# peach-xiao/EMRT

Measured on AMD Instinct MI355X. Metric: training tiles/sec at 256x256, higher is better.
Workload: dtype bf16; 1 GPU; EMRT ResNet50, Potsdam 256x256, 6 classes, batch 8 per GPU, fwd+bwd+SGD step (BASELINE configs[1]), bf16; global_batch=8, parallelism=dp1, hipgraph=True

## Files before the change

emrt_amd/csrc/common.hpp:

```cpp
#pragma once
#include <hip/hip_runtime.h>
#include <stdint.h>
#include <stdio.h>
#include <string.h>

#define EMRT_F32 0
#define EMRT_BF16 1
#define EMRT_F16 2

namespace emrt {

extern thread_local char g_err[512];
inline int fail(const char* fn, const char* msg) {
  snprintf(g_err, sizeof(g_err), "%s: %s", fn, msg);
  return -1;
}
inline int check_launch(const char* fn) {
  hipError_t e = hipGetLastError();
  if (e != hipSuccess) {
    snprintf(g_err, sizeof(g_err), "%s: launch failed: %s", fn, hipGetErrorString(e));
    return -2;
  }
  return 0;
}
#define EMRT_REQUIRE(cond, msg) \
  do {                          \
    if (!(cond)) return emrt::fail(__func__, msg); \
  } while (0)

struct Tuning {
  int conv_tile;
  int wgrad_split;
  int thin_cblk;
  int thin_blocks;
  int thin_ch;
  int no_thin_bwd;
  int igemm64_nst;
  int wgrad_nst;
  int pair_max;
  int msda_fwd_global;
  int msda_bwd_global;
  int msda_lds_min_pairs;
  int msda_bwd_dref_lds;
  int msda_band_halo;
  int msda_scatter_qsplit;
  int msda_scatter_cuts;
  int msda_fwd_chunks;
  int msda_fwd_threads;
  int msda_fwd_probe;
  int bn_block_kb;
  int bn_operand_blocks;
  int ln_bwd_rows;
  int ln_bwd_max_blocks;
  int ln_bwd_threads;
  int ln_atomic;
  int gn_group_blocks;
  int gn_stat_rows;
  int gn_bwd_stat_rows;
  int gn_apply_rows;
  int igemm8p_probe;
  int igemm8p_cmajor;
  int igemm8p_min_blocks;
  int wgrad8p_min_steps;
  int wgrad8p_slab;
  int wgrad8p_xcd;
  int wgrad8p_force;
  int no_ksplit128;
  int wgrad_no_overwrite;
  int no_s2_dgrad;
  int wgroup_blocks;
  int wgroup_min_steps;
  int wgroup_max;
  int wgroup8;
  int wgroup8_blocks;
  int wgroup8_min_work;
  int msda_scatter_merge;
  int msda_scatter_mfma;
  int msda_mf_bands;
  int sgd_nt;
  int mha_bwd_split;
  int mha_valu;
  int no_bna;
  int memcpy_kernel;
  int xk;
};
extern Tuning g_tune;

struct Scratch {
  void* ptr; size_t bytes; void* stream;
  unsigned* tick;
  float* xk_part;
};
constexpr size_t SCRATCH_TICK_BYTES = 65536;
constexpr int SCRATCH_TICKS = (int)(SCRATCH_TICK_BYTES / 4);
constexpr size_t SCRATCH_XK_BYTES = 8u << 20;
extern Scratch g_scratch;

struct bf16_t {
  unsigned short v;
};
struct f16_t {
  unsigned short v;
};

__device__ __forceinline__ float to_f32(float x) { return x; }
__device__ __forceinline__ float to_f32(bf16_t x) { return __uint_as_float(((uint32_t)x.v) << 16); }
__device__ __forceinline__ float to_f32(f16_t x) { return (float)__builtin_bit_cast(_Float16, x.v); }
__device__ __forceinline__ float bf16_bits_to_f32(uint32_t lo16) { return __uint_as_float(lo16 << 16); }
__device__ __forceinline__ float f16_bits_to_f32(uint32_t lo16) { return (float)__builtin_bit_cast(_Float16, (unsigned short)lo16); }

template <class T>
__device__ __forceinline__ T from_f32(float f);
template <>
__device__ __forceinline__ float from_f32<float>(float f) {
  return f;
}
template <>
__device__ __forceinline__ bf16_t from_f32<bf16_t>(float f) {
  __bf16 b = (__bf16)f;
  bf16_t r;
  r.v = __builtin_bit_cast(unsigned short, b);
  return r;
}
template <>
__device__ __forceinline__ f16_t from_f32<f16_t>(float f) {
  f16_t r;
  r.v = __builtin_bit_cast(unsigned short, (_Float16)f);
  return r;
}
typedef __attribute__((ext_vector_type(2))) _Float16 emrt_half2_t;
typedef __attribute__((ext_vector_type(2))) float emrt_float2_t;
__device__ __forceinline__ uint32_t pack_f16x2(float lo, float hi) {
  emrt_half2_t h = __builtin_convertvector((emrt_float2_t){lo, hi}, emrt_half2_t);
  return __builtin_bit_cast(uint32_t, h);
}
__device__ __forceinline__ void unpack_f16x2(uint32_t w, float& lo, float& hi) {
  const emrt_half2_t h = __builtin_bit_cast(emrt_half2_t, w);
  lo = (float)h.x;
  hi = (float)h.y;
}
__device__ __forceinline__ uint32_t pack_bf16x2(float lo, float hi) {
  return (uint32_t)from_f32<bf16_t>(lo).v | ((uint32_t)from_f32<bf16_t>(hi).v << 16);
}

template <class T>
struct Vec4;
template <>
struct Vec4<float> {
  __device__ static __forceinline__ void load(const float* p, float (&o)[4]) {
    float4 v = *reinterpret_cast<const float4*>(p);
    o[0] = v.x; o[1] = v.y; o[2] = v.z; o[3] = v.w;
  }
  __device__ static __forceinline__ void store(float* p, const float (&o)[4]) {
    *reinterpret_cast<float4*>(p) = make_float4(o[0], o[1], o[2], o[3]);
  }
};
template <>
struct Vec4<bf16_t> {
  __device__ static __forceinline__ void load(const bf16_t* p, float (&o)[4]) {
    uint2 v = *reinterpret_cast<const uint2*>(p);
    o[0] = bf16_bits_to_f32(v.x & 0xffffu); o[1] = __uint_as_float(v.x & 0xffff0000u);
    o[2] = bf16_bits_to_f32(v.y & 0xffffu); o[3] = __uint_as_float(v.y & 0xffff0000u);
  }
  __device__ static __forceinline__ void store(bf16_t* p, const float (&o)[4]) {
    uint2 v;
    v.x = pack_bf16x2(o[0], o[1]);
    v.y = pack_bf16x2(o[2], o[3]);
    *reinterpret_cast<uint2*>(p) = v;
  }
};

template <>
struct Vec4<f16_t> {
  __device__ static __forceinline__ void load(const f16_t* p, float (&o)[4]) {
    uint2 v = *reinterpret_cast<const uint2*>(p);
    unpack_f16x2(v.x, o[0], o[1]);
    unpack_f16x2(v.y, o[2], o[3]);
  }
  __device__ static __forceinline__ void store(f16_t* p, const float (&o)[4]) {
    uint2 v;
    v.x = pack_f16x2(o[0], o[1]);
    v.y = pack_f16x2(o[2], o[3]);
    *reinterpret_cast<uint2*>(p) = v;
  }
};

template <class T>
struct Vec8;
template <>
struct Vec8<float> {
  __device__ static __forceinline__ void load(const float* p, float (&o)[8]) {
    float4 a = *reinterpret_cast<const float4*>(p), b = *reinterpret_cast<const float4*>(p + 4);
    o[0] = a.x; o[1] = a.y; o[2] = a.z; o[3] = a.w; o[4] = b.x; o[5] = b.y; o[6] = b.z; o[7] = b.w;
  }
  __device__ static __forceinline__ void store(float* p, const float (&o)[8]) {
    *reinterpret_cast<float4*>(p) = make_float4(o[0], o[1], o[2], o[3]);
    *reinterpret_cast<float4*>(p + 4) = make_float4(o[4], o[5], o[6], o[7]);
  }
};
template <>
struct Vec8<bf16_t> {
  __device__ static __forceinline__ void unpack(const uint4& v, float (&o)[8]) {
    uint32_t w[4] = {v.x, v.y, v.z, v.w};
#pragma unroll
    for (int i = 0; i < 4; ++i) {
      o[2 * i] = bf16_bits_to_f32(w[i] & 0xffffu);
      o[2 * i + 1] = __uint_as_float(w[i] & 0xffff0000u);
    }
  }
  __device__ static __forceinline__ void load(const bf16_t* p, float (&o)[8]) {
    uint4 v = *reinterpret_cast<const uint4*>(p);
    uint32_t w[4] = {v.x, v.y, v.z, v.w};
#pragma unroll
    for (int i = 0; i < 4; ++i) {
      o[2 * i] = bf16_bits_to_f32(w[i] & 0xffffu);
      o[2 * i + 1] = __uint_as_float(w[i] & 0xffff0000u);
    }
  }
  __device__ static __forceinline__ void store(bf16_t* p, const float (&o)[8]) {
    uint4 v;
    v.x = pack_bf16x2(o[0], o[1]); v.y = pack_bf16x2(o[2], o[3]);
    v.z = pack_bf16x2(o[4], o[5]); v.w = pack_bf16x2(o[6], o[7]);
    *reinterpret_cast<uint4*>(p) = v;
  }
};

template <>
struct Vec8<f16_t> {
// ... 92 lines not shown
```

emrt_amd/csrc/conv.hip:

```cpp
#include "common.hpp"
#include "bn_operand.hpp"
#include <stdlib.h>
#include <type_traits>

using namespace emrt;

typedef __attribute__((ext_vector_type(8))) __bf16 bf16x8_t;
typedef __attribute__((ext_vector_type(4))) short short4_t;
typedef __attribute__((ext_vector_type(16))) float f32x16_t;

struct ConvArgs {
  const void* in;
  const void* w;
  void* out;
  const float* bias;
  const float* scale;
  const void* res;
  int N, H, W, C, ldin;
  long long in_bs;
  int OH, OW, OC, ldout;
  long long out_bs;
  int ldres;
  long long res_bs;
  int KH, KW, stride, pad;
// ... 2024 lines not shown
  BwdGroupArgs g;
  bool groupable = true;
  long long total = 0;
  for (int i = 0; i < n; ++i) {
    const EmrtConvBwdDesc& b = descs[i];
    ConvArgs& d = g.d[i];
    d.in = b.dy; d.w = b.w_bwd_packed; d.out = b.dx; d.bias = nullptr; d.scale = nullptr; d.res = b.accumulate ? b.dx : nullptr;
    d.N = b.N; d.H = b.OH; d.W = b.OW; d.C = b.OC; d.ldin = b.lddy; d.in_bs = b.dy_bs;
    d.OH = b.H; d.OW = b.W; d.OC = b.C; d.ldout = b.lddx; d.out_bs = b.dx_bs;
    d.ldres = b.accumulate ? b.lddx : 0; d.res_bs = b.accumulate ? b.dx_bs : 0;
    d.KH = b.KH; d.KW = b.KW; d.stride = b.stride; d.pad = b.pad; d.dil = 1; d.relu = 0; d.out_f32 = 0; d.cmajor = 0; d.stats = nullptr;
    d.mask_y = nullptr; d.ldy = 0; d.y_bs = 0; d.mask_scale = 1.f; d.stat_x = nullptr; d.ldsx = 0; d.sx_bs = 0;
    d.xk_S = 0; d.xk_part = nullptr; d.xk_tick = nullptr; d.drop_seed = nullptr; d.drop_salt = 0; d.drop_p = 0.f;
    WgradArgs& w = g.w[i];
    w.x = b.x; w.dy = b.dy; w.dw = b.dw;
    w.N = b.N; w.H = b.H; w.W = b.W; w.C = b.C; w.ldx = b.ldx; w.x_bs = b.x_bs;
    w.OH = b.OH; w.OW = b.OW; w.OC = b.OC; w.lddy = b.lddy; w.dy_bs = b.dy_bs;
    w.KH = b.KH; w.KW = b.KW; w.stride = b.stride; w.pad = b.pad; w.dil = 1; w.tiles_per_split = 0; w.dbias = b.dbias; w.overwrite = 0;
    const bool vec = conv_desc_is_vec<T>(d) && wgrad_is_vec<T>(w) && d.OC > 32;
    groupable = groupable && vec;
    int tx = 1, ty = 1, S = 1;
    if (vec) wgrad_plan<T>(w, tx, ty, S);
    const long long Md = (long long)d.N * d.OH * d.OW;
    g.nd[i] = (int)(((Md + 63) / 64) * ((d.OC + 63) / 64));
    g.wtx[i] = tx; g.wty[i] = ty;
    g.first[i] = (int)total;
    total += g.nd[i] + (long long)tx * ty * S;
  }
  for (int i = n; i <= EMRT_MAX_GROUP; ++i) g.first[i] = (int)total;
  for (int i = n; i < EMRT_MAX_GROUP; ++i) { g.d[i] = g.d[0]; g.w[i] = g.w[0]; g.nd[i] = 0; g.wtx[i] = 1; g.wty[i] = 1; }
  if (!groupable || total > 4096) {
    for (int i = 0; i < n; ++i) {
      const int rc = conv_bwd_dispatch<T>(g.d[i], g.w[i], st);
      if (rc) return rc;
    }
    return 0;
  }
  auto kern = bwd_group_kernel<T>;
  const size_t lds_d = (size_t)2 * 128 * 144, lds_w = (size_t)4 * Cfg::BKM * Cfg::PITCH;
  const size_t lds = lds_d > lds_w ? lds_d : lds_w;
  static bool attr_done = false;
  if (!attr_done) {
    if (hipFuncSetAttribute(reinterpret_cast<const void*>(kern), hipFuncAttributeMaxDynamicSharedMemorySize, (int)lds) != hipSuccess)
      return fail("emrt_conv2d_bwd_group", "cannot raise the dynamic LDS limit");
    attr_done = true;
  }
  hipLaunchKernelGGL(kern, dim3((unsigned)total), dim3(256), lds, st, g);
  return check_launch("emrt_conv2d_bwd_group");
}

extern "C" int emrt_conv2d_bwd_group(const EmrtConvBwdDesc* descs, int n, int dtype, void* stream) {
  EMRT_REQUIRE(descs && n >= 1 && n <= EMRT_MAX_GROUP, "1..6 problems");
  EMRT_REQUIRE_TRAIN_DTYPE(dtype);
  for (int i = 0; i < n; ++i) {
    const EmrtConvBwdDesc& b = descs[i];
    EMRT_REQUIRE(b.x && b.dy && b.w_bwd_packed && b.dx, "null pointer");
    EMRT_REQUIRE((b.dw == nullptr) == (descs[0].dw == nullptr) && (b.dw || !b.dbias), "dw == NULL (data gradients only) must hold for every problem of the group, without dbias");
    EMRT_REQUIRE(b.N > 0 && b.H > 0 && b.W > 0 && b.C > 0 && b.OC > 0 && b.KH > 0 && b.KW > 0 && b.stride > 0 && b.pad >= 0, "bad dims");
    EMRT_REQUIRE(b.OH == (b.H + 2 * b.pad - b.KH) / b.stride + 1 && b.OW == (b.W + 2 * b.pad - b.KW) / b.stride + 1, "output size mismatch");
    EMRT_REQUIRE((long long)b.N * b.OH * b.OW + 512 < (1ll << 31) && (long long)b.N * b.H * b.W + 512 < (1ll << 31), "more than 2^31 pixels");
    EMRT_REQUIRE(b.lddx >= b.C && b.dx_bs >= 0, "bad dx strides");
    const long long esz = dtype == EMRT_F32 ? 4 : 2;
    const long long x_ext = ((long long)(b.N - 1) * b.x_bs + ((long long)b.H * b.W - 1) * b.ldx + b.C) * esz;
    const long long dy_ext = ((long long)(b.N - 1) * b.dy_bs + ((long long)b.OH * b.OW - 1) * b.lddy + b.OC) * esz;
    EMRT_REQUIRE(b.x_bs >= 0 && b.dy_bs >= 0 && x_ext < (1ll << 31) && dy_ext < (1ll << 31), "operand spans 2 GiB or more");
    EMRT_REQUIRE((long long)b.H * b.W < (1 << 24) && (long long)b.ldx * esz < (1 << 24) && b.stride < (1 << 12), "map too large for the 24-bit address arithmetic");
  }
  hipStream_t st = (hipStream_t)stream;
  return dtype == EMRT_F32 ? conv_bwd_group_dispatch<float>(descs, n, st) : conv_bwd_group_dispatch<bf16_t>(descs, n, st);
}

struct EmrtConvDgradDesc {
  const void* dy; const void* w_bwd_packed; void* dx; int lddx; long long dx_bs; int accumulate;
  int N, H, W, C, OH, OW, OC, lddy; long long dy_bs; int KH, KW, stride, pad, dilation;
  double* bn_stats; const void* mask_y; int ldy; long long y_bs; float mask_scale; const void* stat_x; int ldsx; long long sx_bs;
  const void* addend; int ldadd; long long add_bs;
};

static void dgrad_args_from_desc(ConvArgs& d, const EmrtConvDgradDesc& b) {
  d.in = b.dy; d.w = b.w_bwd_packed; d.out = b.dx; d.bias = nullptr; d.scale = nullptr; d.res = nullptr;
  d.N = b.N; d.H = b.OH; d.W = b.OW; d.C = b.OC; d.ldin = b.lddy; d.in_bs = b.dy_bs;
  d.OH = b.H; d.OW = b.W; d.OC = b.C; d.ldout = b.lddx; d.out_bs = b.dx_bs;
  d.ldres = 0; d.res_bs = 0;
  if (b.accumulate) { d.res = b.dx; d.ldres = b.lddx; d.res_bs = b.dx_bs; }
  else if (b.addend) { d.res = b.addend; d.ldres = b.ldadd; d.res_bs = b.add_bs; }
  d.KH = b.KH; d.KW = b.KW; d.stride = b.stride; d.pad = b.pad; d.dil = b.dilation; d.relu = 0; d.out_f32 = 0; d.cmajor = g_tune.igemm8p_cmajor; d.stats = b.bn_stats;
  d.mask_y = b.mask_y; d.ldy = b.ldy; d.y_bs = b.y_bs; d.mask_scale = b.mask_scale; d.stat_x = b.stat_x; d.ldsx = b.ldsx; d.sx_bs = b.sx_bs;
  d.xk_S = 0; d.xk_part = nullptr; d.xk_tick = nullptr; d.drop_seed = nullptr; d.drop_salt = 0; d.drop_p = 0.f;
}

template <class T>
static int conv_dgrad_multi_dispatch(const EmrtConvDgradDesc* descs, int n, hipStream_t st) {
  ConvGroupArgs g;
  bool groupable = n >= 2;
  long long total = 0;
  for (int i = 0; i < n; ++i) {
    ConvArgs& d = g.p[i];
    dgrad_args_from_desc(d, descs[i]);
    const long long Md = (long long)d.N * d.OH * d.OW;
    const long long nb = ((Md + 63) / 64) * ((d.OC + 63) / 64);
    g.first[i] = (int)total;
    total += nb;
    groupable = groupable && conv_desc_is_vec<T>(d) && d.OC > 32 && nb <= 2048;
  }
  for (int i = n; i <= EMRT_MAX_GROUP; ++i) g.first[i] = (int)total;
  for (int i = n; i < EMRT_MAX_GROUP; ++i) g.p[i] = g.p[0];
  if (!groupable || total > 4096) {
    for (int i = 0; i < n; ++i) {
      const int rc = conv_dispatch<T, 1>(g.p[i], st);
      if (rc) return rc;
    }
    return 0;
  }
  hipLaunchKernelGGL((igemm_group_kernel<T, 1>), dim3((unsigned)total), dim3(256), (size_t)2 * 128 * 144, st, g);
  return check_launch("emrt_conv2d_dgrad_multi");
}

extern "C" int emrt_conv2d_dgrad_multi(const EmrtConvDgradDesc* descs, int n, int dtype, void* stream) {
  EMRT_REQUIRE(descs && n >= 1 && n <= EMRT_MAX_GROUP, "1..6 problems");
  EMRT_REQUIRE_TRAIN_DTYPE(dtype);
  for (int i = 0; i < n; ++i) {
    const EmrtConvDgradDesc& b = descs[i];
    EMRT_REQUIRE(b.dy && b.w_bwd_packed && b.dx, "null pointer");
    EMRT_REQUIRE(b.N > 0 && b.H > 0 && b.W > 0 && b.C > 0 && b.OH > 0 && b.OW > 0 && b.OC > 0, "bad dims");
    EMRT_REQUIRE(b.KH > 0 && b.KW > 0 && b.stride > 0 && b.pad >= 0 && b.dilation >= 1, "bad kernel geometry");
    EMRT_REQUIRE(b.OH == (b.H + 2 * b.pad - b.dilation * (b.KH - 1) - 1) / b.stride + 1 && b.OW == (b.W + 2 * b.pad - b.dilation * (b.KW - 1) - 1) / b.stride + 1, "output size mismatch");
    EMRT_REQUIRE((long long)b.N * b.OH * b.OW + 512 < (1ll << 31) && (long long)b.N * b.H * b.W + 512 < (1ll << 31), "more than 2^31 pixels (32-bit pixel arithmetic)");
    const long long esz = dtype == EMRT_F32 ? 4 : 2;
    const long long dy_ext = ((long long)(b.N - 1) * b.dy_bs + ((long long)b.OH * b.OW - 1) * b.lddy + b.OC) * esz;
    const long long w_ext = (long long)b.OC * b.KH * b.KW * b.C * esz;
    EMRT_REQUIRE(b.dy_bs >= 0 && dy_ext < (1ll << 31) && w_ext < (1ll << 31), "operand spans 2 GiB or more (32-bit buffer offsets)");
    EMRT_REQUIRE((long long)b.OH * b.OW < (1 << 24) && (long long)b.lddy * esz < (1 << 24) && b.stride < (1 << 12), "map too large for the 24-bit address arithmetic");
    EMRT_REQUIRE(b.lddx >= b.C && b.dx_bs >= 0, "bad dx strides");
    EMRT_REQUIRE(!(b.accumulate && b.addend), "accumulate adds into dx itself; addend is a different tensor");
    EMRT_REQUIRE(!b.stat_x || b.mask_y, "stat_x replaces the mask tensor in the second statistic: it needs mask_y");
    for (int j = 0; j < i; ++j) EMRT_REQUIRE(descs[j].dx != b.dx, "two problems of one launch must not write the same dx");
  }
  hipStream_t st = (hipStream_t)stream;
  return dtype == EMRT_F32 ? conv_dgrad_multi_dispatch<float>(descs, n, st) : conv_dgrad_multi_dispatch<bf16_t>(descs, n, st);
}

#define EMRT_MAX_WGROUP 24
struct EmrtWgradDesc {
  const void* x; const void* dy; float* dw; float* dbias;
  int N, H, W, C, ldx; long long x_bs;
  int OH, OW, OC, lddy; long long dy_bs;
  int KH, KW, stride, pad, dilation;
  int dw_is_zero;
};
struct WgradGroupArgs {
  WgradArgs w[EMRT_MAX_WGROUP];
  int first[EMRT_MAX_WGROUP + 1];
  short wtx[EMRT_MAX_WGROUP], wty[EMRT_MAX_WGROUP];
  int n, xcd;
};

template <class T>
__global__ __launch_bounds__(256, 2) void wgrad_group_kernel(WgradGroupArgs g) {
  extern __shared__ __attribute__((aligned(16))) unsigned char smem_all[];
  const int nb = g.first[g.n];
  int w = (int)blockIdx.x;
  if (g.xcd) {
    const int k = w & 7, idx = w >> 3;
    const int w0 = (int)(((long long)k * nb) >> 3), w1 = (int)(((long long)(k + 1) * nb) >> 3);
    w = w0 + idx;
    if (w >= w1) return;
  } else if (w >= nb) return;
  int i = 0;
  for (int k = 1; k < g.n; ++k) i += w >= g.first[k] ? 1 : 0;
  i = __builtin_amdgcn_readfirstlane(i);
  const int local = w - g.first[i];
  const int tx = g.wtx[i], ty = g.wty[i];
  const int bz = __builtin_amdgcn_readfirstlane(local / (tx * ty)), t = __builtin_amdgcn_readfirstlane(local - bz * (tx * ty));
  const int by = __builtin_amdgcn_readfirstlane(t / tx);
  wgrad_body<T, true, 1>(g.w[i], __builtin_amdgcn_readfirstlane(t - by * tx), by, bz, smem_all);
}

static void wgrad_args_from_desc(WgradArgs& a, const EmrtWgradDesc& d) {
  a.x = d.x; a.dy = d.dy; a.dw = d.dw;
  a.N = d.N; a.H = d.H; a.W = d.W; a.C = d.C; a.ldx = d.ldx; a.x_bs = d.x_bs;
  a.OH = d.OH; a.OW = d.OW; a.OC = d.OC; a.lddy = d.lddy; a.dy_bs = d.dy_bs;
  a.KH = d.KH; a.KW = d.KW; a.stride = d.stride; a.pad = d.pad; a.dil = d.dilation; a.tiles_per_split = 0; a.dbias = d.dbias;
  a.overwrite = d.dw_is_zero ? 1 : 0;
}

template <class T>
static int wgrad_group_dispatch(const EmrtWgradDesc* descs, int n, hipStream_t st) {
  using Cfg = WgradCfg<T>;
  WgradArgs pend[EMRT_MAX_WGROUP];
  int npend = 0;
  auto flush = [&]() -> int {
    if (npend == 0) return 0;
    if (npend == 1) { const int rc = wgrad_dispatch<T>(pend[0], st); npend = 0; return rc; }
    int tx[EMRT_MAX_WGROUP], ty[EMRT_MAX_WGROUP], S1[EMRT_MAX_WGROUP];
    long long mt[EMRT_MAX_WGROUP], work = 0;
    for (int i = 0; i < npend; ++i) {
      WgradArgs tmp = pend[i];
      wgrad_plan<T>(tmp, tx[i], ty[i], S1[i]);
      mt[i] = ((long long)pend[i].N * pend[i].OH * pend[i].OW + Cfg::BKM - 1) / Cfg::BKM;
      work += (long long)tx[i] * ty[i] * mt[i];
    }
    int order[EMRT_MAX_WGROUP];
    long long tps[EMRT_MAX_WGROUP], Sl[EMRT_MAX_WGROUP];
    {
      long long Tt = (work + g_tune.wgroup_blocks - 1) / (g_tune.wgroup_blocks > 0 ? g_tune.wgroup_blocks : 1024);
      if (Tt < g_tune.wgroup_min_steps) Tt = g_tune.wgroup_min_steps;
      if (Tt < 1) Tt = 1;
      for (int i = 0; i < npend; ++i) {
        long long S = (mt[i] + Tt - 1) / Tt;
        Sl[i] = S > S1[i] ? S1[i] : (S < 1 ? 1 : S);
      }
    }
    for (int i = 0; i < npend; ++i) {
      tps[i] = (mt[i] + Sl[i] - 1) / Sl[i];
      order[i] = i;
    }
    for (int i = 1; i < npend; ++i)
      for (int j = i; j > 0 && tps[order[j]] > tps[order[j - 1]]; --j) { const int t_ = order[j]; order[j] = order[j - 1]; order[j - 1] = t_; }
    WgradGroupArgs g;
    long long total = 0;
    for (int q = 0; q < npend; ++q) {
      const int i = order[q];
      g.w[q] = pend[i];
      g.w[q].tiles_per_split = (int)tps[i];
      const long long S = (mt[i] + tps[i] - 1) / tps[i];
      if (S > 1 || g_tune.wgrad_no_overwrite) g.w[q].overwrite = 0;
      g.first[q] = (int)total;
      g.wtx[q] = (short)tx[i]; g.wty[q] = (short)ty[i];
      total += (long long)tx[i] * ty[i] * S;
    }
    for (int q = npend; q <= EMRT_MAX_WGROUP; ++q) g.first[q] = (int)total;
    for (int q = npend; q < EMRT_MAX_WGROUP; ++q) { g.w[q] = g.w[0]; g.wtx[q] = 1; g.wty[q] = 1; }
    g.n = npend; g.xcd = g_tune.wgrad8p_xcd;
    npend = 0;
    if (total >= (1ll << 30)) return fail("emrt_conv2d_wgrad_group", "too many blocks");
    auto kern = wgrad_group_kernel<T>;
    const size_t lds = (size_t)4 * Cfg::BKM * Cfg::PITCH;
    static bool attr_done = false;
    if (!attr_done) {
      if (hipFuncSetAttribute(reinterpret_cast<const void*>(kern), hipFuncAttributeMaxDynamicSharedMemorySize, (int)lds) != hipSuccess)
        return fail("emrt_conv2d_wgrad_group", "cannot raise the dynamic LDS limit");
      attr_done = true;
    }
    hipLaunchKernelGGL(kern, dim3(8u * (unsigned)((total + 7) / 8)), dim3(256), lds, st, g);
    return check_launch("emrt_conv2d_wgrad_group");
  };
  WgradArgs pend8[EMRT_MAX_WGROUP8];
  int npend8 = 0;
  auto flush8 = [&]() -> int {
    if (npend8 == 0) return 0;
    const int rc = launch_wgrad8p_group(pend8, npend8, st);
    npend8 = 0;
    return rc;
  };
  auto aliased = [&](int i) { for (int j = 0; j < n; ++j) if (j != i && descs[j].dw == descs[i].dw) return true; return false; };
  long long work8 = 0;
  if constexpr (std::is_same<T, bf16_t>::value) {
    for (int i = 0; i < n && g_tune.wgroup8 > 0; ++i) {
      WgradArgs a;
      wgrad_args_from_desc(a, descs[i]);
      int tk, toc, S8, per, tiles8, steps8;
      if (wgrad_is_vec<T>(a) && !wgrad8p_plan<T>(a, tk, toc, S8, per) && wgrad8p_group_ok<T>(a, tiles8, steps8) && !aliased(i)) work8 += (long long)tiles8 * steps8;
    }
  }
  const bool use8 = g_tune.wgroup8 > 0 && work8 >= (g_tune.wgroup8_min_work > 0 ? g_tune.wgroup8_min_work : 1);
  for (int i = 0; i < n; ++i) {
    WgradArgs a;
    wgrad_args_from_desc(a, descs[i]);
    const bool alias = aliased(i);
    if (alias) a.overwrite = 0;
    bool alone = !wgrad_is_vec<T>(a) || a.KH * a.KW * a.C >= 32768 * 128 || a.OC >= 32768 * 128;
    if constexpr (std::is_same<T, bf16_t>::value) {
      int tk, toc, S8, per;
      if (wgrad8p_plan<T>(a, tk, toc, S8, per)) alone = true;
    }
    if (alone) {
      const int rc = wgrad_dispatch<T>(a, st);
      if (rc) return rc;
      continue;
    }
    if constexpr (std::is_same<T, bf16_t>::value) {
      int tiles8, steps8;
      if (use8 && !alias && wgrad8p_group_ok<T>(a, tiles8, steps8)) {
        pend8[npend8++] = a;
        if (npend8 == EMRT_MAX_WGROUP8) {
          const int rc = flush8();
          if (rc) return rc;
        }
        continue;
      }
    }
    pend[npend++] = a;
    if (npend == EMRT_MAX_WGROUP || (g_tune.wgroup_max > 0 && npend >= g_tune.wgroup_max)) {
      const int rc = flush();
      if (rc) return rc;
    }
  }
  {
    const int rc = flush8();
    if (rc) return rc;
  }
  return flush();
}

extern "C" int emrt_conv2d_wgrad_group(const EmrtWgradDesc* descs, int n, int dtype, void* stream) {
  EMRT_REQUIRE(descs && n >= 1, "no problems");
  EMRT_REQUIRE_TRAIN_DTYPE(dtype);
  for (int i = 0; i < n; ++i) {
    const EmrtWgradDesc& d = descs[i];
    EMRT_REQUIRE(d.x && d.dy && d.dw, "null pointer");
    EMRT_REQUIRE(d.N > 0 && d.H > 0 && d.W > 0 && d.C > 0 && d.OH > 0 && d.OW > 0 && d.OC > 0 && d.dilation >= 1, "bad dims");
    EMRT_REQUIRE(d.KH > 0 && d.KW > 0 && d.stride > 0 && d.pad >= 0, "bad kernel geometry");
    EMRT_REQUIRE(d.OH == (d.H + 2 * d.pad - d.dilation * (d.KH - 1) - 1) / d.stride + 1 && d.OW == (d.W + 2 * d.pad - d.dilation * (d.KW - 1) - 1) / d.stride + 1, "output size mismatch");
    EMRT_REQUIRE((long long)d.N * d.OH * d.OW + 512 < (1ll << 31) && (long long)d.N * d.H * d.W + 512 < (1ll << 31), "more than 2^31 pixels (32-bit pixel arithmetic)");
    const long long esz = dtype == EMRT_F32 ? 4 : 2;
    const long long x_ext = ((long long)(d.N - 1) * d.x_bs + ((long long)d.H * d.W - 1) * d.ldx + d.C) * esz;
    const long long dy_ext = ((long long)(d.N - 1) * d.dy_bs + ((long long)d.OH * d.OW - 1) * d.lddy + d.OC) * esz;
    EMRT_REQUIRE(d.x_bs >= 0 && d.dy_bs >= 0 && x_ext < (1ll << 31) && dy_ext < (1ll << 31), "operand spans 2 GiB or more (32-bit buffer offsets)");
    EMRT_REQUIRE((long long)d.H * d.W < (1 << 24) && (long long)d.ldx * esz < (1 << 24) && d.stride < (1 << 12), "map too large for the 24-bit address arithmetic");
  }
  hipStream_t st = (hipStream_t)stream;
  return dtype == EMRT_F32 ? wgrad_group_dispatch<float>(descs, n, st) : wgrad_group_dispatch<bf16_t>(descs, n, st);
}
```

emrt_amd/csrc/elementwise.hip:

```cpp
#include "common.hpp"
#include <stdlib.h>

using namespace emrt;

thread_local char emrt::g_err[512] = {0};

extern "C" const char* emrt_last_error(void) { return emrt::g_err; }
extern "C" int emrt_abi_version(void) { return 9; }

namespace {
struct TuneEntry { const char* name; int emrt::Tuning::*field; int def; };
const TuneEntry kTune[] = {
    {"conv_tile", &emrt::Tuning::conv_tile, 0},         {"wgrad_split", &emrt::Tuning::wgrad_split, 0},
    {"thin_cblk", &emrt::Tuning::thin_cblk, 64},        {"thin_blocks", &emrt::Tuning::thin_blocks, 128},
    {"thin_ch", &emrt::Tuning::thin_ch, 8},             {"no_thin_bwd", &emrt::Tuning::no_thin_bwd, 0},
    {"pair_max", &emrt::Tuning::pair_max, 768},         {"msda_fwd_global", &emrt::Tuning::msda_fwd_global, 0},
    {"bn_block_kb", &emrt::Tuning::bn_block_kb, 8},     {"ln_atomic", &emrt::Tuning::ln_atomic, 1},
    {"msda_fwd_chunks", &emrt::Tuning::msda_fwd_chunks, 0}, {"msda_fwd_threads", &emrt::Tuning::msda_fwd_threads, 1024},
    {"msda_fwd_probe", &emrt::Tuning::msda_fwd_probe, 0}, {"wgrad_nst", &emrt::Tuning::wgrad_nst, 2},
    {"igemm64_nst", &emrt::Tuning::igemm64_nst, 3}, {"msda_bwd_global", &emrt::Tuning::msda_bwd_global, 0},
    {"msda_lds_min_pairs", &emrt::Tuning::msda_lds_min_pairs, 2048}, {"msda_bwd_dref_lds", &emrt::Tuning::msda_bwd_dref_lds, 1},
    {"gn_group_blocks", &emrt::Tuning::gn_group_blocks, 0}, {"gn_stat_rows", &emrt::Tuning::gn_stat_rows, 32},
    {"gn_bwd_stat_rows", &emrt::Tuning::gn_bwd_stat_rows, 32}, {"gn_apply_rows", &emrt::Tuning::gn_apply_rows, 8},
    {"msda_scatter_cuts", &emrt::Tuning::msda_scatter_cuts, 0}, {"msda_scatter_qsplit", &emrt::Tuning::msda_scatter_qsplit, 0}, {"msda_band_halo", &emrt::Tuning::msda_band_halo, 0},
    {"igemm8p_probe", &emrt::Tuning::igemm8p_probe, 0}, {"igemm8p_min_blocks", &emrt::Tuning::igemm8p_min_blocks, 160}, {"igemm8p_cmajor", &emrt::Tuning::igemm8p_cmajor, 0},
    {"wgrad8p_min_steps", &emrt::Tuning::wgrad8p_min_steps, 8}, {"wgrad8p_slab", &emrt::Tuning::wgrad8p_slab, 1}, {"wgrad8p_force", &emrt::Tuning::wgrad8p_force, 0}, {"wgrad8p_xcd", &emrt::Tuning::wgrad8p_xcd, 1},
    {"wgrad_no_overwrite", &emrt::Tuning::wgrad_no_overwrite, 0}, {"no_ksplit128", &emrt::Tuning::no_ksplit128, 0}, {"ln_bwd_rows", &emrt::Tuning::ln_bwd_rows, 0}, {"ln_bwd_max_blocks", &emrt::Tuning::ln_bwd_max_blocks, 0}, {"bn_operand_blocks", &emrt::Tuning::bn_operand_blocks, 0}, {"no_s2_dgrad", &emrt::Tuning::no_s2_dgrad, 0}, {"wgroup_blocks", &emrt::Tuning::wgroup_blocks, 1024}, {"wgroup_min_steps", &emrt::Tuning::wgroup_min_steps, 32}, {"wgroup_max", &emrt::Tuning::wgroup_max, 0},
    {"no_bna", &emrt::Tuning::no_bna, 0}, {"memcpy_kernel", &emrt::Tuning::memcpy_kernel, 0}, {"xk", &emrt::Tuning::xk, 0}, {"mha_valu", &emrt::Tuning::mha_valu, 0}, {"mha_bwd_split", &emrt::Tuning::mha_bwd_split, 1}, {"msda_scatter_merge", &emrt::Tuning::msda_scatter_merge, 0},
    {"wgroup8", &emrt::Tuning::wgroup8, 0}, {"wgroup8_blocks", &emrt::Tuning::wgroup8_blocks, 0}, {"wgroup8_min_work", &emrt::Tuning::wgroup8_min_work, 6000},
    {"msda_scatter_mfma", &emrt::Tuning::msda_scatter_mfma, 1}, {"sgd_nt", &emrt::Tuning::sgd_nt, 1}, {"ln_bwd_threads", &emrt::Tuning::ln_bwd_threads, 512}, {"msda_mf_bands", &emrt::Tuning::msda_mf_bands, 0},
};
emrt::Tuning tuning_from_env() {
  emrt::Tuning t;
  for (const TuneEntry& e : kTune) {
    char env[64] = "EMRT_";
    size_t n = strlen(env);
    for (const char* c = e.name; *c && n + 1 < sizeof(env); ++c) env[n++] = (char)((*c >= 'a' && *c <= 'z') ? *c - 32 : *c);
    env[n] = 0;
    const char* v = (strcmp(e.name, "msda_fwd_probe") == 0 || strcmp(e.name, "igemm8p_probe") == 0) ? nullptr : getenv(env);
    t.*(e.field) = v ? atoi(v) : e.def;
  }
  return t;
}
}
emrt::Tuning emrt::g_tune = tuning_from_env();
emrt::Scratch emrt::g_scratch = {nullptr, 0, nullptr, nullptr, nullptr};

extern "C" int emrt_set_scratch(void* ptr, size_t bytes, void* stream) {
  EMRT_REQUIRE((ptr != nullptr) == (bytes > 0) && ((uintptr_t)ptr) % 256 == 0, "scratch must be 256-byte aligned device memory (or nullptr, 0)");
  if (ptr && ptr == emrt::g_scratch.ptr && emrt::g_scratch.tick && bytes == emrt::g_scratch.bytes + emrt::SCRATCH_TICK_BYTES + emrt::SCRATCH_XK_BYTES) {
    emrt::g_scratch.stream = stream;
    return 0;
  }
  emrt::g_scratch.ptr = ptr;
  emrt::g_scratch.bytes = bytes;
  emrt::g_scratch.stream = stream;
  emrt::g_scratch.tick = nullptr;
  emrt::g_scratch.xk_part = nullptr;
  if (ptr && bytes >= (16u << 20) + emrt::SCRATCH_XK_BYTES + emrt::SCRATCH_TICK_BYTES && bytes % 256 == 0) {
    emrt::g_scratch.bytes = bytes - emrt::SCRATCH_TICK_BYTES - emrt::SCRATCH_XK_BYTES;
    emrt::g_scratch.xk_part = reinterpret_cast<float*>(static_cast<char*>(ptr) + emrt::g_scratch.bytes);
    emrt::g_scratch.tick = reinterpret_cast<unsigned*>(static_cast<char*>(ptr) + emrt::g_scratch.bytes + emrt::SCRATCH_XK_BYTES);
    if (hipMemsetAsync(emrt::g_scratch.tick, 0, emrt::SCRATCH_TICK_BYTES, (hipStream_t)stream) != hipSuccess) {
      emrt::g_scratch.tick = nullptr;
      return emrt::fail("emrt_set_scratch", "cannot zero the arrival counters");
    }
  }
  return 0;
}

extern "C" int emrt_set_tuning(const char* name, int value) {
  EMRT_REQUIRE(name, "null name");
  for (const TuneEntry& e : kTune)
    if (strcmp(e.name, name) == 0) { emrt::g_tune.*(e.field) = value; return 0; }
  return emrt::fail("emrt_set_tuning", "unknown knob");
}
extern "C" int emrt_get_tuning(const char* name, int* value) {
  EMRT_REQUIRE(name && value, "null pointer");
  for (const TuneEntry& e : kTune)
    if (strcmp(e.name, name) == 0) { *value = emrt::g_tune.*(e.field); return 0; }
  return emrt::fail("emrt_get_tuning", "unknown knob");
}

static inline int ew_grid(long long total) {
  long long g = (total + 255) / 256;
  if (g > 8192) g = 8192;
  if (g < 1) g = 1;
  return (int)g;
}

template <class T>
__global__ __launch_bounds__(256) void add_kernel(const T* __restrict__ a, const T* __restrict__ b, T* __restrict__ out, long long n4,
                                                  long long period4) {
  for (long long i = (long long)blockIdx.x * blockDim.x + threadIdx.x; i < n4; i += (long long)gridDim.x * blockDim.x) {
    float x[4], y[4];
    Vec4<T>::load(a + i * 4, x);
    Vec4<T>::load(b + ((n4 | period4) <= 0xffffffffll ? (long long)((unsigned)i % (unsigned)period4) : i % period4) * 4, y);
#pragma unroll
    for (int e = 0; e < 4; ++e) x[e] += y[e];
    Vec4<T>::store(out + i * 4, x);
  }
}

template <class T>
__global__ __launch_bounds__(256) void add_f32row_kernel(const T* __restrict__ a, const float* __restrict__ b, T* __restrict__ out,
                                                         long long n4, long long period4) {
  for (long long i = (long long)blockIdx.x * blockDim.x + threadIdx.x; i < n4; i += (long long)gridDim.x * blockDim.x) {
    float x[4];
    Vec4<T>::load(a + i * 4, x);
    const float4 y = reinterpret_cast<const float4*>(b)[(n4 | period4) <= 0xffffffffll ? (long long)((unsigned)i % (unsigned)period4) : i % period4];
    x[0] += y.x; x[1] += y.y; x[2] += y.z; x[3] += y.w;
    Vec4<T>::store(out + i * 4, x);
  }
}

struct LevelStarts { int start[5]; int L; };
template <class T>
__global__ __launch_bounds__(256) void add_f32row_levels_kernel(const T* __restrict__ a, const float* __restrict__ rows, T* __restrict__ out,
                                                                long long n4, int C4, LevelStarts ls) {
  for (long long i = (long long)blockIdx.x * blockDim.x + threadIdx.x; i < n4; i += (long long)gridDim.x * blockDim.x) {
    const int r = (int)(i / C4), c4 = (int)(i - (long long)r * C4);
    int l = 0;
#pragma unroll
    for (int k = 1; k < 4; ++k) l += (k < ls.L && r >= ls.start[k]) ? 1 : 0;
    float x[4];
    Vec4<T>::load(a + i * 4, x);
    const float4 y = reinterpret_cast<const float4*>(rows)[(long long)l * C4 + c4];
    x[0] += y.x; x[1] += y.y; x[2] += y.z; x[3] += y.w;
    Vec4<T>::store(out + i * 4, x);
  }
}

template <class T>
__global__ __launch_bounds__(256) void acc3d_kernel(T* __restrict__ dst, long long dst_bs, long long dst_rs, const T* __restrict__ src,
                                                    long long src_bs, long long src_rs, long long B, long long rows, long long cols4) {
  const long long total = B * rows * cols4;
  for (long long i = (long long)blockIdx.x * blockDim.x + threadIdx.x; i < total; i += (long long)gridDim.x * blockDim.x) {
    int c4, ri;
    long long b;
    unravel3(i, (int)cols4, (int)rows, total <= 0xffffffffll, c4, ri, b);
    const long long c = (long long)c4 * 4, r = ri;
    float x[4], y[4];
    Vec4<T>::load(dst + b * dst_bs + r * dst_rs + c, x);
    Vec4<T>::load(src + b * src_bs + r * src_rs + c, y);
#pragma unroll
    for (int e = 0; e < 4; ++e) x[e] += y[e];
    Vec4<T>::store(dst + b * dst_bs + r * dst_rs + c, x);
  }
}

template <class T>
__global__ __launch_bounds__(256) void add3d_kernel(const T* __restrict__ a, long long a_bs, long long a_rs, const T* __restrict__ b2,
                                                    long long b_bs, long long b_rs, T* __restrict__ out, long long o_bs, long long o_rs,
                                                    long long B, long long rows, long long cols4) {
  const long long total = B * rows * cols4;
  for (long long i = (long long)blockIdx.x * blockDim.x + threadIdx.x; i < total; i += (long long)gridDim.x * blockDim.x) {
    int c4, ri;
    long long b;
    unravel3(i, (int)cols4, (int)rows, total <= 0xffffffffll, c4, ri, b);
    const long long c = (long long)c4 * 4, r = ri;
    float x[4], y[4];
    Vec4<T>::load(a + b * a_bs + r * a_rs + c, x);
    Vec4<T>::load(b2 + b * b_bs + r * b_rs + c, y);
#pragma unroll
    for (int e = 0; e < 4; ++e) x[e] += y[e];
    Vec4<T>::store(out + b * o_bs + r * o_rs + c, x);
  }
}

template <class T>
__global__ __launch_bounds__(256) void dropout_fwd_kernel(const T* __restrict__ x, T* __restrict__ y, long long n4, float p,
                                                          const unsigned long long* __restrict__ seed, unsigned salt, int mode,
                                                          long long hw, int C) {
  const unsigned long long sd = seed[0];
  const float ks = 1.f / (1.f - p);
  for (long long i = (long long)blockIdx.x * blockDim.x + threadIdx.x; i < n4; i += (long long)gridDim.x * blockDim.x) {
    float v[4];
    Vec4<T>::load(x + i * 4, v);
    if (mode == 0) {
      uint32_t h[2];
      drop_quad(sd, salt, (unsigned long long)i, h);
      const uint32_t thr = drop_thr16(p);
// ... 295 lines not shown
```

Before: 1009 tiles/s.

## Pair two wgrad tiles per 512-thread block sharing an LDS operand

Adds a grouped weight-gradient kernel in which each 512-thread block runs two 256-thread halves on adjacent output tiles. When both tiles use the same x slice or the same dy slice, only one copy of that operand is staged in LDS, which cuts global loads and LDS stores for that operand. Tile pairing order is chosen so that pairs tend to share a row or column, and it is enabled by default for bf16. The cost is double the LDS per block, one block per CU, tiles of a pair run in lockstep, and more complex bias reduction.

```diff
diff --git a/emrt_amd/csrc/common.hpp b/emrt_amd/csrc/common.hpp
--- a/emrt_amd/csrc/common.hpp
+++ b/emrt_amd/csrc/common.hpp
@@ -74,6 +74,7 @@
   int wgroup8;
   int wgroup8_blocks;
   int wgroup8_min_work;
+  int wgroup_pair;
   int msda_scatter_merge;
   int msda_scatter_mfma;
   int msda_mf_bands;
diff --git a/emrt_amd/csrc/conv.hip b/emrt_amd/csrc/conv.hip
--- a/emrt_amd/csrc/conv.hip
+++ b/emrt_amd/csrc/conv.hip
@@ -2200,6 +2200,8 @@
   WgradArgs w[EMRT_MAX_WGROUP];
   int first[EMRT_MAX_WGROUP + 1];
   short wtx[EMRT_MAX_WGROUP], wty[EMRT_MAX_WGROUP];
+  short wS[EMRT_MAX_WGROUP];
+  unsigned char word[EMRT_MAX_WGROUP];
   int n, xcd;
 };
 
@@ -2224,6 +2226,254 @@
   wgrad_body<T, true, 1>(g.w[i], __builtin_amdgcn_readfirstlane(t - by * tx), by, bz, smem_all);
 }
 
+template <int NSTW, int MODE>
+__device__ __forceinline__ void wgrad_pair_body(const WgradArgs& p, const int bx0, const int by0, const int bz0, const int bx1, const int by1, const int bz1,
+                                                const bool act1, unsigned char* smem_all) {
+  using T = bf16_t;
+  using Cfg = WgradCfg<T>;
+  constexpr int EPC = 8, CPR = Cfg::CPR, RPP = Cfg::RPP, BKM = Cfg::BKM, PITCH = Cfg::PITCH;
+  constexpr int NST = NSTW;
+  constexpr int TILE_BYTES = BKM * PITCH, BUF_BYTES = 4 * TILE_BYTES;
+
+  const int grp = __builtin_amdgcn_readfirstlane((int)threadIdx.x >> 8);
+  const int tid = threadIdx.x & 255, lane = tid & 63, wave = tid >> 6;
+  const int wr = wave >> 1, wc = wave & 1;
+  const bool active = grp == 0 || act1;
+  const int block_x = grp ? bx1 : bx0, block_y = grp ? by1 : by0, block_z = grp ? bz1 : bz0;
+  constexpr bool share_x = MODE == 1, share_dy = MODE == 2;
+  constexpr int NP = share_dy ? 2 : 4, NQ = share_x ? 2 : 4;
+  const int offP = (share_dy ? 0 : 2 * grp) * TILE_BYTES, offQ = (share_x ? 1 : 2 * grp + 1) * TILE_BYTES;
+
+  const int K = p.KH * p.KW * p.C;
+  const int oc0 = block_y * 128, k0 = block_x * 128;
+  const __amdgpu_buffer_rsrc_t rs_x = __builtin_amdgcn_make_buffer_rsrc((void*)p.x, 0, (int)BUF_RANGE, 0x00020000);
+  const __amdgpu_buffer_rsrc_t rs_dy = __builtin_amdgcn_make_buffer_rsrc((void*)p.dy, 0, (int)BUF_RANGE, 0x00020000);
+
+  const int col = tid % CPR, prow = tid / CPR;
+  const int kq = k0 + col * EPC;
+  const int tap = kq < K ? kq / p.C : 0;
+  const int cq = kq - tap * p.C;
+  const int kh = tap / p.KW, kw = tap - kh * p.KW;
+  const int ocp = oc0 + col * EPC;
+  const unsigned q_bad = kq < K ? 0u : BUF_OOB;
+  const unsigned p_bad = ocp < p.OC ? 0u : BUF_OOB;
+
+  f32x16_t acc[2][2];
+#pragma unroll
+  for (int i = 0; i < 2; ++i)
+#pragma unroll
+    for (int j = 0; j < 2; ++j)
+#pragma unroll
+      for (int r = 0; r < 16; ++r) acc[i][j][r] = 0.f;
+
+  const long long mt_total = ((long long)p.N * p.OH * p.OW + BKM - 1) / BKM;
+  auto slice_len = [&](int bz) {
+    long long n = mt_total - (long long)bz * p.tiles_per_split;
+    if (n > p.tiles_per_split) n = p.tiles_per_split;
+    return n < 0 ? 0 : (int)n;
+  };
+  const int nt0 = slice_len(bz0), nt1 = act1 ? slice_len(bz1) : 0;
+  const int ntile = grp ? nt1 : nt0;
+  const int niter = nt0 > nt1 ? nt0 : nt1;
+  if (niter <= 0) return;
+  const long long mt_begin = (long long)block_z * p.tiles_per_split;
+
+  constexpr unsigned ESZ = (unsigned)sizeof(T);
+  int r_nb[4], r_oh[4], r_ow[4];
+  unsigned r_dy[4], r_ximg[4];
+  {
+    const int OHW = p.OH * p.OW;
+#pragma unroll
+    for (int i = 0; i < 4; ++i) {
+      const unsigned m = (unsigned)(mt_begin * BKM) + (unsigned)(prow + RPP * ((i + 2 * grp) & 3));
+      r_nb[i] = (int)(m / (unsigned)OHW);
+      const int pix = (int)(m - (unsigned)r_nb[i] * (unsigned)OHW);
+      r_oh[i] = (int)((unsigned)pix / (unsigned)p.OW);
+      r_ow[i] = pix - r_oh[i] * p.OW;
+      r_dy[i] = (unsigned)(((long long)r_nb[i] * p.dy_bs + (long long)pix * p.lddy) * (long long)ESZ);
+      r_ximg[i] = (unsigned)((long long)r_nb[i] * p.x_bs * (long long)ESZ);
+    }
+  }
+  const int adv_w = BKM % p.OW, adv_q = BKM / p.OW;
+  const int adv_h = adv_q % p.OH, adv_n = adv_q / p.OH;
+  const unsigned dy_step = (unsigned)BKM * (unsigned)p.lddy * ESZ;
+  const unsigned dy_wrap = (unsigned)((p.dy_bs - (long long)p.OH * p.OW * p.lddy) * (long long)ESZ);
+  const unsigned x_bs_b = (unsigned)(p.x_bs * (long long)ESZ);
+  const unsigned dy_adv = dy_step + (unsigned)adv_n * dy_wrap, x_adv = (unsigned)adv_n * x_bs_b;
+  const unsigned ldx_b = (unsigned)p.ldx * ESZ, cq_b = (unsigned)cq * ESZ, ocp_b = (unsigned)ocp * ESZ;
+  const int hi0 = kh * p.dil - p.pad, wi0 = kw * p.dil - p.pad;
+  int ld_t = 0;
+
+  uint4 rp[NST][NP], rq[NST][NQ];
+  auto load_tile = [&](uint4 (&rp_)[NP], uint4 (&rq_)[NQ]) {
+    const unsigned t_bad = ld_t < ntile ? 0u : BUF_OOB;
+    ld_t += 1;
+#pragma unroll
+    for (int i = 0; i < 4; ++i) {
+      const unsigned m_bad = (r_nb[i] < p.N ? 0u : BUF_OOB) | t_bad;
+      {
+        if (i < NP) rp_[i < NP ? i : 0] = buf_load16(rs_dy, (r_dy[i] | m_bad | p_bad) + ocp_b);
+        if (i < NQ) {
+          const int hi = __mul24(r_oh[i], p.stride) + hi0, wi = __mul24(r_ow[i], p.stride) + wi0;
+          const bool inb = (unsigned)hi < (unsigned)p.H && (unsigned)wi < (unsigned)p.W;
+          const unsigned off = r_ximg[i] + __umul24((unsigned)(__mul24(hi, p.W) + wi), ldx_b) + cq_b;
+          rq_[i < NQ ? i : 0] = buf_load16(rs_x, inb ? (off | m_bad | q_bad) : BUF_OOB);
+        }
+      }
+      r_ow[i] += adv_w;
+      const int c1 = r_ow[i] >= p.OW ? 1 : 0;
+      r_ow[i] -= c1 ? p.OW : 0;
+      r_oh[i] += adv_h + c1;
+      const int c2 = r_oh[i] >= p.OH ? 1 : 0;
+      r_oh[i] -= c2 ? p.OH : 0;
+      r_nb[i] += adv_n + c2;
+      r_dy[i] += dy_adv + (c2 ? dy_wrap : 0u);
+      r_ximg[i] += x_adv + (c2 ? x_bs_b : 0u);
+    }
+  };
+
+  const bool sum_bias = p.dbias != nullptr && active && (share_dy ? bx0 == 0 : block_x == 0);
+  const bool any_bias = p.dbias != nullptr && (bx0 == 0 || (act1 && bx1 == 0));
+  float bsum[EPC];
+#pragma unroll
+  for (int e = 0; e < EPC; ++e) bsum[e] = 0.f;
+
+  auto m_tile = [&](uint4 (&rp_)[NP], uint4 (&rq_)[NQ], int par, bool refill, int tcur) {
+    unsigned char* sP = smem_all + par * BUF_BYTES + offP;
+    unsigned char* sQ = smem_all + par * BUF_BYTES + offQ;
+    const bool live = tcur < ntile;
+#pragma unroll
+    for (int i = 0; i < NP; ++i) *reinterpret_cast<uint4*>(sP + (prow + RPP * ((i + 2 * grp) & 3)) * PITCH + col * 16) = rp_[i];
+#pragma unroll
+    for (int i = 0; i < NQ; ++i) *reinterpret_cast<uint4*>(sQ + (prow + RPP * ((i + 2 * grp) & 3)) * PITCH + col * 16) = rq_[i];
+    if (sum_bias) {
+#pragma unroll
+      for (int i = 0; i < NP; ++i) {
+        const uint32_t w4[4] = {rp_[i].x, rp_[i].y, rp_[i].z, rp_[i].w};
+#pragma unroll
+        for (int e = 0; e < EPC; ++e) bsum[e] += bf16_bits_to_f32((w4[e >> 1] >> (16 * (e & 1))) & 0xffffu);
+      }
+    }
+    __syncthreads();
+    if (refill) load_tile(rp_, rq_);
+    if (!live) return;
+    const int g = lane >> 4, t = lane & 15;
+    const int h = g >> 1, half = g & 1, q = t >> 2, pp = t & 3;
+#pragma unroll
+    for (int s = 0; s < BKM / 16; ++s) {
+      uint4 fa[2], fb[2];
+      const int r0 = 16 * s + 8 * h + q;
+#pragma unroll
+      for (int i = 0; i < 2; ++i) {
+        const int cb = (wr * 64 + i * 32 + 16 * half + 4 * pp) * 2;
+        short4_t lo = __builtin_amdgcn_ds_read_tr16_b64_v4i16((__attribute__((address_space(3))) short4_t*)(sP + r0 * PITCH + cb));
+        short4_t hi = __builtin_amdgcn_ds_read_tr16_b64_v4i16((__attribute__((address_space(3))) short4_t*)(sP + (r0 + 4) * PITCH + cb));
+        uint2 l2 = __builtin_bit_cast(uint2, lo), h2 = __builtin_bit_cast(uint2, hi);
+        fa[i] = make_uint4(l2.x, l2.y, h2.x, h2.y);
+      }
+#pragma unroll
+      for (int j = 0; j < 2; ++j) {
+        const int cb = (wc * 64 + j * 32 + 16 * half + 4 * pp) * 2;
+        short4_t lo = __builtin_amdgcn_ds_read_tr16_b64_v4i16((__attribute__((address_space(3))) short4_t*)(sQ + r0 * PITCH + cb));
+        short4_t hi = __builtin_amdgcn_ds_read_tr16_b64_v4i16((__attribute__((address_space(3))) short4_t*)(sQ + (r0 + 4) * PITCH + cb));
+        uint2 l2 = __builtin_bit_cast(uint2, lo), h2 = __builtin_bit_cast(uint2, hi);
+        fb[j] = make_uint4(l2.x, l2.y, h2.x, h2.y);
+      }
+#pragma unroll
+      for (int i = 0; i < 2; ++i)
+#pragma unroll
+        for (int j = 0; j < 2; ++j)
+          acc[i][j] = __builtin_amdgcn_mfma_f32_32x32x16_bf16(__builtin_bit_cast(bf16x8_t, fa[i]), __builtin_bit_cast(bf16x8_t, fb[j]), acc[i][j], 0, 0, 0);
+    }
+  };
+
+#pragma unroll
+  for (int d = 0; d < NST; ++d) load_tile(rp[d], rq[d]);
+  int t = 0;
+  for (; t + NST <= niter; t += NST) {
+#pragma unroll
+    for (int d = 0; d < NST; ++d) m_tile(rp[d], rq[d], (t + d) & 1, true, t + d);
+  }
+  const int rem = niter - t;
+#pragma unroll
+  for (int d = 0; d < NST - 1; ++d)
+    if (d < rem) m_tile(rp[d], rq[d], (t + d) & 1, false, t + d);
+  __syncthreads();
+
+  if (any_bias) {
+    float* sb = reinterpret_cast<float*>(smem_all);
+#pragma unroll
+    for (int e = 0; e < EPC; ++e) sb[(grp * RPP + prow) * 128 + col * EPC + e] = bsum[e];
+    __syncthreads();
+    if (sum_bias && (!share_dy || grp == 0) && tid < 128 && oc0 + tid < p.OC) {
+      const int rb = share_dy ? 0 : grp * RPP, nr = share_dy ? 2 * RPP : RPP;
+      float tsum = 0.f;
+      for (int r = 0; r < nr; ++r) tsum += sb[(rb + r) * 128 + tid];
+      atomicAdd(p.dbias + oc0 + tid, tsum);
+    }
+  }
+  if (!active) return;
+  const int frow = lane & 31, fh = lane >> 5;
+#pragma unroll
+  for (int i = 0; i < 2; ++i)
+#pragma unroll
+    for (int r = 0; r < 16; ++r) {
+      const int oc = oc0 + wr * 64 + i * 32 + (r & 3) + 8 * (r >> 2) + 4 * fh;
+      if (oc >= p.OC) continue;
+#pragma unroll
+      for (int j = 0; j < 2; ++j) {
+        const int k = k0 + wc * 64 + j * 32 + frow;
+        if (k < K) {
+          if (p.overwrite) p.dw[(long long)oc * K + k] = acc[i][j][r];
+          else atomicAdd(p.dw + (long long)oc * K + k, acc[i][j][r]);
+        }
+      }
+    }
+}
+
+template <int NSTW>
+__global__ __launch_bounds__(512, 1) void wgrad_pair_group_kernel(WgradGroupArgs g) {
+  extern __shared__ __attribute__((aligned(16))) unsigned char smem_all[];
+  const int nb = g.first[g.n];
+  int w = (int)blockIdx.x;
+  if (g.xcd) {
+    const int k = w & 7, idx = w >> 3;
+    const int w0 = (int)(((long long)k * nb) >> 3), w1 = (int)(((long long)(k + 1) * nb) >> 3);
+    w = w0 + idx;
+    if (w >= w1) return;
+  } else if (w >= nb) return;
+  int i = 0;
+  for (int k = 1; k < g.n; ++k) i += w >= g.first[k] ? 1 : 0;
+  i = __builtin_amdgcn_readfirstlane(i);
+  const int local = w - g.first[i];
+  const int tx = g.wtx[i], ty = g.wty[i], tt = tx * ty;
+  int bx[2], by[2], bz[2];
+  bool act1;
+  if (tt == 1) {
+    bx[0] = bx[1] = by[0] = by[1] = 0;
+    bz[0] = 2 * local; bz[1] = 2 * local + 1;
+    act1 = bz[1] < (int)g.wS[i];
+  } else {
+    const int pps = (tt + 1) >> 1;
+    const int z = __builtin_amdgcn_readfirstlane(local / pps), q = local - z * pps;
+    act1 = 2 * q + 1 < tt;
+#pragma unroll
+    for (int h = 0; h < 2; ++h) {
+      const int t = (h && act1) ? 2 * q + 1 : 2 * q;
+      const int d = g.word[i] ? tx : ty;
+      const int hi = __builtin_amdgcn_readfirstlane(t / d), lo = t - hi * d;
+      bx[h] = g.word[i] ? lo : hi;
+      by[h] = g.word[i] ? hi : lo;
+      bz[h] = z;
+    }
+  }
+  if (!act1) bz[1] = bz[0];
+  const bool same_slice = act1 && bz[0] == bz[1];
+  if (same_slice && bx[0] == bx[1]) wgrad_pair_body<NSTW, 1>(g.w[i], bx[0], by[0], bz[0], bx[1], by[1], bz[1], act1, smem_all);
+  else if (same_slice && by[0] == by[1]) wgrad_pair_body<NSTW, 2>(g.w[i], bx[0], by[0], bz[0], bx[1], by[1], bz[1], act1, smem_all);
+  else wgrad_pair_body<NSTW, 0>(g.w[i], bx[0], by[0], bz[0], bx[1], by[1], bz[1], act1, smem_all);
+}
+
 static void wgrad_args_from_desc(WgradArgs& a, const EmrtWgradDesc& d) {
   a.x = d.x; a.dy = d.dy; a.dw = d.dw;
   a.N = d.N; a.H = d.H; a.W = d.W; a.C = d.C; a.ldx = d.ldx; a.x_bs = d.x_bs;
@@ -2265,6 +2515,7 @@
     }
     for (int i = 1; i < npend; ++i)
       for (int j = i; j > 0 && tps[order[j]] > tps[order[j - 1]]; --j) { const int t_ = order[j]; order[j] = order[j - 1]; order[j - 1] = t_; }
+    const bool pair = std::is_same<T, bf16_t>::value && g_tune.wgroup_pair > 0;
     WgradGroupArgs g;
     long long total = 0;
     for (int q = 0; q < npend; ++q) {
@@ -2275,13 +2526,30 @@
       if (S > 1 || g_tune.wgrad_no_overwrite) g.w[q].overwrite = 0;
       g.first[q] = (int)total;
       g.wtx[q] = (short)tx[i]; g.wty[q] = (short)ty[i];
-      total += (long long)tx[i] * ty[i] * S;
+      g.wS[q] = (short)S;
+      g.word[q] = ty[i] % 2 == 0 ? 0 : 1;
+      const long long tt = (long long)tx[i] * ty[i];
+      total += !pair ? tt * S : tt == 1 ? (S + 1) / 2 : ((tt + 1) / 2) * S;
     }
     for (int q = npend; q <= EMRT_MAX_WGROUP; ++q) g.first[q] = (int)total;
-    for (int q = npend; q < EMRT_MAX_WGROUP; ++q) { g.w[q] = g.w[0]; g.wtx[q] = 1; g.wty[q] = 1; }
+    for (int q = npend; q < EMRT_MAX_WGROUP; ++q) { g.w[q] = g.w[0]; g.wtx[q] = 1; g.wty[q] = 1; g.wS[q] = 1; g.word[q] = 0; }
     g.n = npend; g.xcd = g_tune.wgrad8p_xcd;
     npend = 0;
     if (total >= (1ll << 30)) return fail("emrt_conv2d_wgrad_group", "too many blocks");
+    if constexpr (std::is_same<T, bf16_t>::value) {
+      if (pair) {
+        const size_t lds2 = (size_t)2 * 4 * Cfg::BKM * Cfg::PITCH;
+        static bool attr2_done = false;
+        if (!attr2_done) {
+          if (hipFuncSetAttribute(reinterpret_cast<const void*>(wgrad_pair_group_kernel<2>), hipFuncAttributeMaxDynamicSharedMemorySize, (int)lds2) != hipSuccess)
+            return fail("emrt_conv2d_wgrad_group", "cannot raise the dynamic LDS limit");
+          attr2_done = true;
+        }
+        const dim3 grid2(8u * (unsigned)((total + 7) / 8));
+        hipLaunchKernelGGL(wgrad_pair_group_kernel<2>, grid2, dim3(512), lds2, st, g);
+        return check_launch("emrt_conv2d_wgrad_group");
+      }
+    }
     auto kern = wgrad_group_kernel<T>;
     const size_t lds = (size_t)4 * Cfg::BKM * Cfg::PITCH;
     static bool attr_done = false;
diff --git a/emrt_amd/csrc/elementwise.hip b/emrt_amd/csrc/elementwise.hip
--- a/emrt_amd/csrc/elementwise.hip
+++ b/emrt_amd/csrc/elementwise.hip
@@ -27,7 +27,7 @@
     {"wgrad8p_min_steps", &emrt::Tuning::wgrad8p_min_steps, 8}, {"wgrad8p_slab", &emrt::Tuning::wgrad8p_slab, 1}, {"wgrad8p_force", &emrt::Tuning::wgrad8p_force, 0}, {"wgrad8p_xcd", &emrt::Tuning::wgrad8p_xcd, 1},
     {"wgrad_no_overwrite", &emrt::Tuning::wgrad_no_overwrite, 0}, {"no_ksplit128", &emrt::Tuning::no_ksplit128, 0}, {"ln_bwd_rows", &emrt::Tuning::ln_bwd_rows, 0}, {"ln_bwd_max_blocks", &emrt::Tuning::ln_bwd_max_blocks, 0}, {"bn_operand_blocks", &emrt::Tuning::bn_operand_blocks, 0}, {"no_s2_dgrad", &emrt::Tuning::no_s2_dgrad, 0}, {"wgroup_blocks", &emrt::Tuning::wgroup_blocks, 1024}, {"wgroup_min_steps", &emrt::Tuning::wgroup_min_steps, 32}, {"wgroup_max", &emrt::Tuning::wgroup_max, 0},
     {"no_bna", &emrt::Tuning::no_bna, 0}, {"memcpy_kernel", &emrt::Tuning::memcpy_kernel, 0}, {"xk", &emrt::Tuning::xk, 0}, {"mha_valu", &emrt::Tuning::mha_valu, 0}, {"mha_bwd_split", &emrt::Tuning::mha_bwd_split, 1}, {"msda_scatter_merge", &emrt::Tuning::msda_scatter_merge, 0},
-    {"wgroup8", &emrt::Tuning::wgroup8, 0}, {"wgroup8_blocks", &emrt::Tuning::wgroup8_blocks, 0}, {"wgroup8_min_work", &emrt::Tuning::wgroup8_min_work, 6000},
+    {"wgroup8", &emrt::Tuning::wgroup8, 0}, {"wgroup8_blocks", &emrt::Tuning::wgroup8_blocks, 0}, {"wgroup8_min_work", &emrt::Tuning::wgroup8_min_work, 6000}, {"wgroup_pair", &emrt::Tuning::wgroup_pair, 1},
     {"msda_scatter_mfma", &emrt::Tuning::msda_scatter_mfma, 1}, {"sgd_nt", &emrt::Tuning::sgd_nt, 1}, {"ln_bwd_threads", &emrt::Tuning::ln_bwd_threads, 512}, {"msda_mf_bands", &emrt::Tuning::msda_mf_bands, 0},
 };
 emrt::Tuning tuning_from_env() {
```

New measurement: 995.1 tiles/s. 0.986x the previous value.
